# jmhb0/view_neti

Hardware: AMD Instinct MI355X
Metric: TI train steps/sec (SD-1.5 512^2 bs=4 per GPU) (higher is better)
Workload: dtype f16; 1 GPU; learnable_mode 0, sd15 shapes, 512x512 fp16, bs=4/GPU, grad_accum 1, full train step (VAE+16xCLIP+UNet fwd/bwd+AdamW); global_batch=4, parallelism=dp1, rccl_ranks=1, hipgraph=True

## Files before the change

### view_neti_amd/csrc/gemm8.hip

```cpp
#include <type_traits>

#include "common.h"
#include "gemm_args.h"

namespace {

constexpr int BM = 256, NT = 512;
constexpr int HALF_BYTES = 128 * 128;
constexpr int GN_IMG = 5;

#define VN_WAIT_VM(n) asm volatile("s_waitcnt vmcnt(" #n ")" ::: "memory")
#define VN_WAIT_LGKM0() asm volatile("s_waitcnt lgkmcnt(0)" ::: "memory")

template <int BN, int EPI, bool CONV, bool HALO = false>
__global__ __launch_bounds__(NT) void gemm8_kernel(GemmArgs g) {
  static_assert(BN == 256 || BN == 128, "tile width");
  static_assert(!HALO || (BN == 128 && CONV), "the halo-patch loop exists for the 256x128 convolution tile");
  constexpr int PATCH_STRIDE = 41 * 1024;
  constexpr bool H42 = HALO && BN == 128;
  constexpr int NJB = BN / 128;
  constexpr int HB_BYTES = (BN / 2) * 128;
  constexpr int HB_DMA = BN / 128;
  constexpr int NBUF = BN == 256 ? 2 : 3;
  constexpr int BUF_BYTES = 2 * HALF_BYTES + 2 * HB_BYTES;
  constexpr int CS_LD = BN + 8;
  constexpr int CS_BYTES = BM * CS_LD * 2;
  constexpr int LOOP_BYTES = HALO ? 2 * PATCH_STRIDE + 3 * 2 * HB_BYTES : NBUF * BUF_BYTES;
  constexpr int LDS_BYTES = CS_BYTES > LOOP_BYTES ? CS_BYTES : LOOP_BYTES;
  constexpr int GN_NG = BN / 4 + 2;
  const half_t* const e_gate = EPI == 2 ? g.gate_src : nullptr;
  half_t* const e_C2 = EPI == 2 ? g.C2 : nullptr;
  const int e_geglu = EPI == 2 ? g.geglu : 0;
  const int e_act = EPI == 2 ? g.act : 0;
  float* const e_gn_sums = EPI >= 1 ? g.gn_sums : nullptr;
  const half_t* const e_rowadd = EPI >= 1 ? g.rowadd : nullptr;
  const int e_conv = CONV ? g.conv_mode : 0;
  constexpr int GN_BYTES = EPI == 0 ? 0 : GN_IMG * GN_NG * 4 * 8;
  __shared__ __attribute__((aligned(16))) char smem[LDS_BYTES + GN_BYTES];

  const int tid = threadIdx.x;
  const int lane = tid & 63;
  const int wave = __builtin_amdgcn_readfirstlane(tid >> 6);
  const int wr = wave >> 2, wc = wave & 3;

  int nblk = g.tiles_m * g.tiles_n;
  int bid = blockIdx.x;
  {
    int q = nblk >> 3, r = nblk & 7, xcd = bid & 7, idx = bid >> 3;
    bid = (xcd < r ? xcd * (q + 1) : r * (q + 1) + (xcd - r) * q) + idx;
  }
  const int tile_m = bid / g.tiles_n;
  const int tile_n = bid - tile_m * g.tiles_n;
  const int m0 = tile_m * BM;
  const int n0 = tile_n * BN;
  const int bz = blockIdx.y;
  const int kz = blockIdx.z;
  int hb = 0, hty = 0, htx = 0, row0 = m0;
  if constexpr (HALO) {
    const int tpr = g.Wo >> 4, tpi = (g.Ho >> 4) * tpr;
    hb = tile_m / tpi;
    const int rem = tile_m - hb * tpi;
    hty = rem / tpr;
    htx = rem - hty * tpr;
    row0 = (hb * g.Ho + hty * 16) * g.Wo + htx * 16;
  }
  auto rowmem = [&](const int r) { return HALO ? row0 + (r >> 4) * g.Wo + (r & 15) : m0 + r; };

  const half_t* Ab = g.A + (long long)bz * g.strideA;
  const half_t* Bb = g.B + (long long)bz * g.strideB;
  const __amdgpu_buffer_rsrc_t rsA = vn_make_rsrc(Ab, g.a_bytes);
  const __amdgpu_buffer_rsrc_t rsB = vn_make_rsrc(Bb, g.b_bytes);

  const int lrow = tid >> 3;
  const int gchunk = (tid & 7) ^ ((lrow >> 1) & 7);
  const float rcp_hw = CONV ? 1.0f / (float)(g.Ho * g.Wo) : 0.f, rcp_wo = CONV ? 1.0f / (float)g.Wo : 0.f;
  int a_base[4];
  uint32_t a_mask[4];
#pragma unroll
  for (int r = 0; r < (HALO ? 0 : 4); ++r) {
    const int m = m0 + (r >> 1) * 128 + (r & 1) * 64 + lrow;
    const bool ok = m < g.M;
    if constexpr (!CONV) {
      a_base[r] = (int)((long long)m * g.lda * 2) + gchunk * 16;
      a_mask[r] = ok ? 1u : 0u;
    } else {
      const int hw = g.Ho * g.Wo;
      int b = (int)((float)m * rcp_hw);
      int rem = m - b * hw;
      if (rem < 0) { b -= 1; rem += hw; } else if (rem >= hw) { b += 1; rem -= hw; }
      int oy = (int)((float)rem * rcp_wo);
      int ox = rem - oy * g.Wo;
      if (ox < 0) { oy -= 1; ox += g.Wo; } else if (ox >= g.Wo) { oy += 1; ox -= g.Wo; }
      const int py = e_conv == 1 ? oy * g.stride - g.pad_t : oy + g.pad_t;
      const int px = e_conv == 1 ? ox * g.stride - g.pad_l : ox + g.pad_l;
      a_base[r] = ((b * g.Hi + py) * g.Wi + px) * g.ldx2 + gchunk * 16;
      const int sgn = e_conv == 1 ? 1 : -1;
      uint32_t colbits = 0, mask = 0;
#pragma unroll
      for (int d = 0; d < 3; ++d) colbits |= ((unsigned)(px + sgn * d) < (unsigned)g.Wi ? 1u : 0u) << d;
#pragma unroll
      for (int d = 0; d < 3; ++d) mask |= ((unsigned)(py + sgn * d) < (unsigned)g.Hi ? colbits : 0u) << (3 * d);
      a_mask[r] = ok ? mask : 0u;
    }
  }
  uint32_t b_base[4];
#pragma unroll
  for (int r = 0; r < 4; ++r) {
    const int n = n0 + (r >> 1) * (BN / 2) + (r & 1) * 64 + lrow;
    b_base[r] = (n < g.N) ? (uint32_t)((long long)n * g.ldb * 2) + gchunk * 16 : VN_OOB;
  }

  const int nk_total = g.K / 64;
  const int kt_begin = kz * g.kt_per_split;
  const int kt_end = min(nk_total, kt_begin + g.kt_per_split);
  const int T = kt_end - kt_begin;

  int a_kt[2] = {kt_begin, kt_begin}, b_kt[2] = {kt_begin, kt_begin};
  int a_tap[2], a_ci0[2];
  {
    int tap = 0, ci0 = 0;
    if constexpr (CONV) {
      if (g.korder) {
        ci0 = (kt_begin / 9) * 64;
        tap = kt_begin - (kt_begin / 9) * 9;
      } else {
        tap = (kt_begin * 64) / g.Ci;
        ci0 = kt_begin * 64 - tap * g.Ci;
      }
    }
    a_tap[0] = a_tap[1] = tap;
    a_ci0[0] = a_ci0[1] = ci0;
  }
  const int tap_step = (e_conv == 2 ? -1 : 1) * g.ldx2;
  uint32_t nxt[4];
  auto prepA = [&](const int h) {
    const bool live = a_kt[h] < kt_end;
    int soff;
    uint32_t tapbit;
    if constexpr (!CONV) {
      soff = a_kt[h] * 128;
      tapbit = live ? 1u : 0u;
    } else {
      const int tap = a_tap[h];
      const int dy = (tap * 11) >> 5;
      const int dx = tap - 3 * dy;
      soff = (dy * g.Wi + dx) * tap_step + a_ci0[h] * 2;
      tapbit = live ? (1u << tap) : 0u;
      if (g.korder) {
        a_tap[h] += 1;
        if (a_tap[h] == 9) {
          a_tap[h] = 0;
          a_ci0[h] += 64;
        }
      } else {
        a_ci0[h] += 64;
        if (a_ci0[h] == g.Ci) {
          a_ci0[h] = 0;
          a_tap[h] += 1;
        }
      }
    }
#pragma unroll
    for (int j = 0; j < 2; ++j) {
      nxt[j] = (a_mask[2 * h + j] & tapbit) ? (uint32_t)(a_base[2 * h + j] + soff) : VN_OOB;
    }
    a_kt[h] += 1;
  };
  auto prepB = [&](const int h) {
    const bool live = b_kt[h] < kt_end;
    const uint32_t soff = (uint32_t)b_kt[h] * 128u, dead = live ? 0u : VN_OOB;
    if constexpr (BN == 256) {
#pragma unroll
      for (int j = 0; j < 2; ++j) nxt[j] = (b_base[2 * h + j] + soff) | dead;
    } else {
      nxt[2 + h] = (b_base[2 * h] + soff) | dead;
    }
    b_kt[h] += 1;
  };
  auto issueA = [&](const int h, const int buf) {
    char* dst = smem + buf * BUF_BYTES + h * HALF_BYTES + wave * 1024;
#pragma unroll
    for (int j = 0; j < 2; ++j)
      dma16(rsA, dst + j * 8192, nxt[j]);
  };
  auto issueB = [&](const int h, const int buf) {
    char* dst = smem + buf * BUF_BYTES + 2 * HALF_BYTES + h * HB_BYTES + wave * 1024;
    if constexpr (BN == 256) {
#pragma unroll
      for (int j = 0; j < 2; ++j) dma16(rsB, dst + j * 8192, nxt[j]);
    } else {
      dma16(rsB, dst, nxt[2 + h]);
    }
  };

  const int frow = lane & 15;
  const int fq = lane >> 4;
  const int fkey = (frow >> 1) & 7;
  int rdA[2], rdB[2];
#pragma unroll
  for (int s = 0; s < 2; ++s) {
    const int ch = ((s * 4 + fq) ^ fkey) << 4;
    rdA[s] = (wr * 64 + frow) * 128 + ch;
    rdB[s] = 2 * HALF_BYTES + (wc * (16 * NJB) + frow) * 128 + ch;
  }
  half8 af[4][2], bf0[NJB][2], bf1[NJB][2];
  auto readA = [&](const int h) {
#pragma unroll
    for (int i = 0; i < 4; ++i)
#pragma unroll
      for (int s = 0; s < 2; ++s)
        af[i][s] = as_half8(*reinterpret_cast<const u32x4*>(smem + rdA[s] + h * HALF_BYTES + i * 2048));
  };
  auto readB0 = [&](const int flip) {
#pragma unroll
    for (int jb = 0; jb < NJB; ++jb)
#pragma unroll
      for (int s = 0; s < 2; ++s)
        bf0[jb][s] = as_half8(*reinterpret_cast<const u32x4*>(smem + (rdB[s] ^ flip) + jb * 2048));
  };
  auto readB1 = [&]() {
#pragma unroll
    for (int jb = 0; jb < NJB; ++jb)
#pragma unroll
      for (int s = 0; s < 2; ++s)
        bf1[jb][s] = as_half8(*reinterpret_cast<const u32x4*>(smem + rdB[s] + HB_BYTES + jb * 2048));
  };

  const int wr4 = wave >> 1, wc2 = wave & 1;
  auto acc_row = [&](const int h, const int i) { return H42 ? wr4 * 64 + i * 16 + frow : h * 128 + wr * 64 + i * 16 + frow; };
  auto acc_col = [&](const int h, const int j, const int jb) {
    return H42 ? wc2 * 64 + (2 * h + j) * 16 + 4 * fq : j * (BN / 2) + wc * (16 * NJB) + jb * 16 + 4 * fq;
  };
  f32x4 bv[H42 ? 2 : 1][2][NJB];
  {
    const __amdgpu_buffer_rsrc_t rsBias = vn_make_rsrc(g.bias, g.bias ? (uint32_t)g.N * 4u : 0u);
#pragma unroll
    for (int h = 0; h < (H42 ? 2 : 1); ++h)
#pragma unroll
      for (int j = 0; j < 2; ++j)
#pragma unroll
        for (int jb = 0; jb < NJB; ++jb)
          bv[h][j][jb] = __builtin_bit_cast(f32x4, vn_buf_load16(rsBias, (uint32_t)(n0 + acc_col(h, j, jb)) * 4u));
  }
  f32x4 acc[2][2][4][NJB];
#pragma unroll
  for (int h = 0; h < 2; ++h)
#pragma unroll
    for (int j = 0; j < 2; ++j)
#pragma unroll
      for (int i = 0; i < 4; ++i)
#pragma unroll
        for (int jb = 0; jb < NJB; ++jb) acc[h][j][i][jb] = f32x4{0.f, 0.f, 0.f, 0.f};

#define VN_MMA(H, J, BF, PREP)                                                                                 \
  do {                                                                                                         \
    VN_WAIT_LGKM0();                                                                                           \
    __builtin_amdgcn_s_setprio(1);                                                                             \
    PREP;                                                                                                      \
    _Pragma("unroll") for (int s = 0; s < 2; ++s) _Pragma("unroll") for (int i = 0; i < 4; ++i)                \
        _Pragma("unroll") for (int jb = 0; jb < NJB; ++jb) acc[H][J][i][jb] =                                  \
            VN_MFMA_16x16x32(BF[jb][s], af[i][s], acc[H][J][i][jb], 0, 0, 0);                                  \
    __builtin_amdgcn_s_setprio(0);                                                                             \
  } while (0)
#define VN_PHASE_SYNC()                    \
  do {                                     \
    VN_WAIT_VM(10);                        \
    __builtin_amdgcn_s_barrier();          \
    __builtin_amdgcn_sched_barrier(0);     \
  } while (0)
#define VN_PHASE_END()                     \
  do {                                     \
    __builtin_amdgcn_s_barrier();          \
    __builtin_amdgcn_sched_barrier(0);     \
  } while (0)

#define VN_MMA2(H, PREP)                                                                                       \
  do {                                                                                                         \
    VN_WAIT_LGKM0();                                                                                           \
    __builtin_amdgcn_s_setprio(1);                                                                             \
    PREP;                                                                                                      \
    _Pragma("unroll") for (int s = 0; s < 2; ++s) _Pragma("unroll") for (int i = 0; i < 4; ++i) {              \
      acc[H][0][i][0] = VN_MFMA_16x16x32(bf0[0][s], af[i][s], acc[H][0][i][0], 0, 0, 0);                       \
      acc[H][1][i][0] = VN_MFMA_16x16x32(bf1[0][s], af[i][s], acc[H][1][i][0], 0, 0, 0);                       \
    }                                                                                                          \
    __builtin_amdgcn_s_setprio(0);                                                                             \
  } while (0)
#define VN_SYNC(n)                         \
  do {                                     \
    VN_WAIT_VM(n);                         \
    __builtin_amdgcn_s_barrier();          \
    __builtin_amdgcn_sched_barrier(0);     \
  } while (0)
  if constexpr (HALO) {
    constexpr int BRING = 2 * PATCH_STRIDE;
    auto patch_key = [](const int px) { return (int)((0x270745032ull >> (4 * (px >> 1))) & 7); };
    constexpr int PROW = 18 * 128;
    const int c_begin = kt_begin / 9, c_end = kt_end / 9;
    uint32_t pa_off[6];
#pragma unroll
    for (int j = 0; j < 6; ++j) {
      const int q = (j * 8 + wave) * 64 + lane, p = q >> 3, cs = q & 7;
      const int py = (p * 3641) >> 16;
      const int px = p - py * 18;
      const int iy = hty * 16 + py - 1, ix = htx * 16 + px - 1;
      const bool ok = p < 324 && (unsigned)iy < (unsigned)g.Hi && (unsigned)ix < (unsigned)g.Wi;
      pa_off[j] = ok ? (uint32_t)(((hb * g.Hi + iy) * g.Wi + ix) * g.ldx2 + ((cs ^ patch_key(px)) << 4)) : VN_OOB;
    }
    const int np_wave = wave == 0 ? 6 : 5;
    auto issueP = [&](const int j, const int chunk) {
      dma16(rsA, smem + (chunk & 1) * PATCH_STRIDE + (j * 8 + wave) * 1024, pa_off[j] + (uint32_t)chunk * 128u);
    };
    auto tap_dy = [&](const int tap) { const int dy = (tap * 11) >> 5; return e_conv == 2 ? 2 - dy : dy; };
    auto tap_dx = [&](const int tap) { const int dx = tap - 3 * ((tap * 11) >> 5); return e_conv == 2 ? 2 - dx : dx; };
    {
      constexpr int BBUF = 2 * HB_BYTES;
      auto issueBt = [&](const int kt, const int buf) {
        const uint32_t soff = (uint32_t)(kt_begin + kt) * 128u, dead = kt < T ? 0u : VN_OOB;
        char* dst = smem + BRING + buf * BBUF + wave * 1024;
        dma16(rsB, dst, (b_base[0] + soff) | dead);
        dma16(rsB, dst + HB_BYTES, (b_base[2] + soff) | dead);
      };
      int lb[3];
#pragma unroll
      for (int dx = 0; dx < 3; ++dx) lb[dx] = (wr4 * 4) * PROW + (frow + dx) * 128 + ((fq ^ patch_key(frow + dx)) << 4);
      const int rb0 = (wc2 * 64 + frow) * 128 + ((fq ^ fkey) << 4);
      half8 bfh[4][2];
      auto readAh = [&](const int half, const int ab) {
#pragma unroll
        for (int i = 2 * half; i < 2 * half + 2; ++i) {
          af[i][0] = as_half8(*reinterpret_cast<const u32x4*>(smem + ab + i * PROW));
          af[i][1] = as_half8(*reinterpret_cast<const u32x4*>(smem + (ab ^ 64) + i * PROW));
        }
      };
#define VN_MMA4(HALF, PREP)                                                                                    \
  do {                                                                                                         \
    VN_WAIT_LGKM0();                                                                                           \
    __builtin_amdgcn_s_setprio(1);                                                                             \
    PREP;                                                                                                      \
    _Pragma("unroll") for (int s = 0; s < 2; ++s) _Pragma("unroll") for (int i = 2 * HALF; i < 2 * HALF + 2; ++i) \
        _Pragma("unroll") for (int cb = 0; cb < 4; ++cb) {                                                     \
      acc[cb >> 1][cb & 1][i][0] =                                                                             \
          VN_MFMA_16x16x32(bfh[cb][s], af[i][s], acc[cb >> 1][cb & 1][i][0], 0, 0, 0);                         \
    }                                                                                                          \
    __builtin_amdgcn_s_setprio(0);                                                                             \
  } while (0)
      int abt[9];
#pragma unroll
      for (int k = 0; k < 9; ++k) {
        const int tp = e_conv == 2 ? 8 - k : k, dy = tp / 3, dx = tp - 3 * dy;
        abt[k] = (dx == 0 ? lb[0] : (dx == 1 ? lb[1] : lb[2])) + dy * PROW + (c_begin & 1) * PATCH_STRIDE;
      }
      uint32_t bo0 = b_base[0] + (uint32_t)(kt_begin + 2) * 128u, bo1 = b_base[2] + (uint32_t)(kt_begin + 2) * 128u;
      uint32_t pp[6];
#pragma unroll
      for (int j = 0; j < 6; ++j) pp[j] = pa_off[j] + (uint32_t)(c_begin + 1) * 128u;
      const bool w0 = wave == 0;
      char* const bring = smem + BRING + wave * 1024;
      auto readBh = [&](const int slot) {
        const char* b = smem + BRING + slot * BBUF;
#pragma unroll
        for (int cb = 0; cb < 4; ++cb) {
          bfh[cb][0] = as_half8(*reinterpret_cast<const u32x4*>(b + cb * 2048 + rb0));
          bfh[cb][1] = as_half8(*reinterpret_cast<const u32x4*>(b + cb * 2048 + (rb0 ^ 64)));
        }
      };
#pragma unroll
      for (int j = 0; j < 6; ++j)
        if (j < np_wave) issueP(j, c_begin);
      issueBt(0, 0);
      issueBt(1, 1);
      VN_WAIT_VM(2);
      __builtin_amdgcn_s_barrier();
      __builtin_amdgcn_sched_barrier(0);
      if (wr == 1) __builtin_amdgcn_s_barrier();
      __builtin_amdgcn_sched_barrier(0);
      auto ktile = [&](auto tap_c, const bool last_chunk, const int pslot) {
        constexpr int tap = decltype(tap_c)::value;
        constexpr int rslot = tap % 3, sslot = (tap + 2) % 3;
        const int ab = abt[tap];
        readBh(rslot);
        readAh(0, ab);
        if constexpr (tap >= 1 && tap <= 6) {
          if (tap < 6 || w0) {
            dma16(rsA, smem + pslot + ((tap - 1) * 8) * 1024 + wave * 1024, last_chunk ? VN_OOB : pp[tap - 1]);
          }
        }
        {
          const uint32_t dead = (last_chunk && tap >= 7) ? VN_OOB : 0u;
          dma16(rsB, bring + sslot * BBUF, bo0 | dead);
          dma16(rsB, bring + sslot * BBUF + HB_BYTES, bo1 | dead);
          bo0 += 128u;
          bo1 += 128u;
        }
        __builtin_amdgcn_s_barrier();
        __builtin_amdgcn_sched_barrier(0);
        VN_MMA4(0, (void)0);
        VN_PHASE_END();
        readAh(1, ab);
        if constexpr (tap >= 1 && tap <= 5) {
          VN_SYNC(3);
        } else if constexpr (tap == 6) {
          if (w0) {
            VN_SYNC(3);
          } else {
            VN_SYNC(2);
          }
        } else {
          VN_SYNC(2);
        }
        VN_MMA4(1, (void)0);
        VN_PHASE_END();
      };
      for (int c = c_begin; c < c_end; ++c) {
        const bool last_chunk = c + 1 >= c_end;
        const int pslot = ((c + 1) & 1) * PATCH_STRIDE;
        ktile(std::integral_constant<int, 0>{}, last_chunk, pslot);
        ktile(std::integral_constant<int, 1>{}, last_chunk, pslot);
        ktile(std::integral_constant<int, 2>{}, last_chunk, pslot);
        ktile(std::integral_constant<int, 3>{}, last_chunk, pslot);
        ktile(std::integral_constant<int, 4>{}, last_chunk, pslot);
        ktile(std::integral_constant<int, 5>{}, last_chunk, pslot);
        ktile(std::integral_constant<int, 6>{}, last_chunk, pslot);
        ktile(std::integral_constant<int, 7>{}, last_chunk, pslot);
        ktile(std::integral_constant<int, 8>{}, last_chunk, pslot);
        const int flip = (c & 1) ? -PATCH_STRIDE : PATCH_STRIDE;
#pragma unroll
        for (int k = 0; k < 9; ++k) abt[k] += flip;
#pragma unroll
        for (int j = 0; j < 6; ++j) pp[j] += 128u;
      }
#undef VN_MMA4
    }
  } else if constexpr (BN == 256) {
    prepB(0);
    issueB(0, 0);
    prepA(0);
    issueA(0, 0);
    prepB(1);
    issueB(1, 0);
    prepA(1);
    issueA(1, 0);
    prepB(0);
    issueB(0, 1);
    prepA(0);
    issueA(0, 1);
    prepB(1);
    issueB(1, 1);
    prepA(1);
    VN_WAIT_VM(10);
    __builtin_amdgcn_s_barrier();
    __builtin_amdgcn_sched_barrier(0);
    readB0(0);
    VN_WAIT_LGKM0();
    __builtin_amdgcn_sched_barrier(0);
    if (wr == 1) __builtin_amdgcn_s_barrier();
    __builtin_amdgcn_sched_barrier(0);

    int cur = 0;
    for (int t = 0; t < T; ++t) {
      readA(0);
      issueA(1, cur ^ 1);
      VN_PHASE_SYNC();
      VN_MMA(0, 0, bf0, prepB(0));
      VN_PHASE_END();
      readB1();
      issueB(0, cur);
      VN_PHASE_SYNC();
      VN_MMA(0, 1, bf1, prepA(0));
      VN_PHASE_END();
      readA(1);
      issueA(0, cur);
      VN_PHASE_SYNC();
      VN_MMA(1, 0, bf0, prepB(1));
      VN_PHASE_END();
      readB0(BUF_BYTES);
      issueB(1, cur);
      VN_PHASE_SYNC();
      VN_MMA(1, 1, bf1, prepA(1));
      VN_PHASE_END();
      cur ^= 1;
#pragma unroll
      for (int s = 0; s < 2; ++s) {
        rdA[s] ^= BUF_BYTES;
        rdB[s] ^= BUF_BYTES;
      }
    }
  } else {
#pragma unroll
    for (int t0 = 0; t0 < 2; ++t0) {
      prepA(0);
      prepB(0);
      prepB(1);
      issueA(0, t0);
      issueB(0, t0);
      issueB(1, t0);
      prepA(1);
      issueA(1, t0);
    }
    prepA(0);
    prepB(0);
    prepB(1);
    VN_WAIT_VM(8);
    __builtin_amdgcn_s_barrier();
    __builtin_amdgcn_sched_barrier(0);
    if (wr == 1) __builtin_amdgcn_s_barrier();
    __builtin_amdgcn_sched_barrier(0);
    int stg = 2;
    for (int t = 0; t < T; ++t) {
      readB0(0);
      readB1();
      readA(0);
      issueA(0, stg);
      issueB(0, stg);
      issueB(1, stg);
      VN_SYNC(10);
      VN_MMA2(0, prepA(1));
      VN_PHASE_END();
      readA(1);
      issueA(1, stg);
      VN_SYNC(8);
      VN_MMA2(1, (prepA(0), prepB(0), prepB(1)));
      VN_PHASE_END();
      stg = stg == 2 ? 0 : stg + 1;
#pragma unroll
      for (int s = 0; s < 2; ++s) {
        rdA[s] = rdA[s] >= 2 * BUF_BYTES ? rdA[s] - 2 * BUF_BYTES : rdA[s] + BUF_BYTES;
        rdB[s] = rdB[s] >= 2 * BUF_BYTES ? rdB[s] - 2 * BUF_BYTES : rdB[s] + BUF_BYTES;
      }
    }
#undef VN_MMA2
#undef VN_SYNC
  }
  if (wr == 0) __builtin_amdgcn_s_barrier();
  asm volatile("s_waitcnt vmcnt(0) lgkmcnt(0)" ::: "memory");
  __syncthreads();
#undef VN_MMA
#undef VN_PHASE_SYNC
#undef VN_PHASE_END

  if (g.ksplit > 1) {
    float* ws = g.ws + ((long long)(kz * g.batch + bz) * g.M) * g.N;
    const __amdgpu_buffer_rsrc_t rsW = vn_make_rsrc(ws, 0x7fffffffu);
#pragma unroll
    for (int h = 0; h < 2; ++h)
#pragma unroll
      for (int j = 0; j < 2; ++j)
#pragma unroll
        for (int i = 0; i < 4; ++i)
#pragma unroll
          for (int jb = 0; jb < NJB; ++jb) {
            const int m = rowmem(acc_row(h, i));
            const int n = n0 + acc_col(h, j, jb);
            if (m < g.M && n < g.N) {
              float* p = ws + (long long)m * g.N + n;
              if (n + 4 <= g.N && (g.N & 3) == 0) {
                vn_st16_wt(rsW, (uint32_t)(((long long)m * g.N + n) * 4), acc[h][j][i][jb]);
              } else {
                for (int e = 0; e < 4 && n + e < g.N; ++e) p[e] = acc[h][j][i][jb][e];
              }
            }
          }
    return;
  }

  if (e_gn_sums && !(HALO && g.gn_hw == g.Ho * g.Wo)) {
    vn_u64* gacc = reinterpret_cast<vn_u64*>(smem + LDS_BYTES);
    for (int i = tid; i < GN_IMG * GN_NG * 4; i += NT) gacc[i] = 0;
  }
  {
    const int nsw = ((frow >> 3) & 1) << 2;
#pragma unroll
    for (int h = 0; h < 2; ++h)
#pragma unroll
      for (int i = 0; i < 4; ++i)
#pragma unroll
        for (int j = 0; j < 2; ++j)
#pragma unroll
          for (int jb = 0; jb < NJB; ++jb) {
            const int ml = acc_row(h, i);
            const int nl = acc_col(h, j, jb) ^ nsw;
            half4 o;
#pragma unroll
            for (int e = 0; e < 4; ++e)
              o[e] = (half_t)apply_act(acc[h][j][i][jb][e] * g.alpha + bv[H42 ? h : 0][j][jb][e], e_act);
            *reinterpret_cast<half4*>(smem + ((size_t)ml * CS_LD + nl) * 2) = o;
          }
  }
  __syncthreads();

  half_t* Cb = reinterpret_cast<half_t*>(g.C) + (long long)bz * g.strideC;
  const __amdgpu_buffer_rsrc_t rsC = vn_make_rsrc(Cb, 0x7fffffffu);
  const __amdgpu_buffer_rsrc_t rsC2 = vn_make_rsrc(e_C2, e_C2 ? 0x7fffffffu : 0u);
  const half_t* Rb = reinterpret_cast<const half_t*>(g.resid);
  if (Rb) Rb += (long long)bz * g.strideC;
  constexpr int CPR = BN / 8;
  constexpr int U = EPI == 2 ? 2 : (EPI == 1 ? 4 : (BN == 256 ? 8 : 4));
  static_assert(NT % CPR == 0 && CPR <= 32 && (BM * CPR) % NT == 0, "a thread keeps one 8-column chunk over all its rows");
  vn_u64* gacc = reinterpret_cast<vn_u64*>(smem + LDS_BYTES);
  const bool gn = e_gn_sums != nullptr;
  const float rcp_gnhw = gn ? 1.0f / (float)g.gn_hw : 0.f, rcp_rpg = e_rowadd ? 1.0f / (float)g.rows_per_group : 0.f;
  const int gn_img0 = gn ? row0 / g.gn_hw : 0, gn_g0t = gn ? n0 / g.gn_cpg : 0;
  const int c = (tid % CPR) * 8;
  const int n = n0 + c;
  const int gn_glo = gn ? n / g.gn_cpg : 0;
  const int gn_split = gn ? (gn_glo + 1) * g.gn_cpg - n : 8;
  int gn_img = -1;
  float s_lo = 0.f, q_lo = 0.f, s_hi = 0.f, q_hi = 0.f;
  auto gn_flush = [&]() {
    const int iref = __builtin_amdgcn_readfirstlane(gn_img);
    const bool uni = __all(gn_img == iref) && iref >= 0;
    if (uni) {
#pragma unroll
      for (int off = 32; off >= CPR; off >>= 1) {
        s_lo += __shfl_xor(s_lo, off);
        q_lo += __shfl_xor(q_lo, off);
        s_hi += __shfl_xor(s_hi, off);
        q_hi += __shfl_xor(q_hi, off);
      }
    }
    if (gn_img >= 0 && (!uni || lane < CPR)) {
      vn_u64* a = gacc + ((gn_img - gn_img0) * GN_NG + (gn_glo - gn_g0t)) * 4;
      vn_fx_add2(a, s_lo, q_lo);
      if (gn_split < 8) vn_fx_add2(a + 4, s_hi, q_hi);
    }
    s_lo = q_lo = s_hi = q_hi = 0.f;
  };
  const bool full_chunk = n + 8 <= g.N;
  const bool swap_halves = ((tid / CPR) >> 3) & 1;
  const __amdgpu_buffer_rsrc_t rsR = vn_make_rsrc(Rb, Rb ? 0x7fffffffu : 0u);
  const __amdgpu_buffer_rsrc_t rsRA = vn_make_rsrc(e_rowadd, e_rowadd ? 0x7fffffffu : 0u);
  const __amdgpu_buffer_rsrc_t rsG = vn_make_rsrc(e_gate, e_gate ? 0x7fffffffu : 0u);
  const int r_first = tid / CPR;
  constexpr int RPP = NT / CPR;
  const bool gn_one = HALO && gn && g.gn_hw == g.Ho * g.Wo;
  const bool ra_one = HALO && EPI >= 1 && e_rowadd && g.rows_per_group == g.Ho * g.Wo;
  half8 av_tile = half8{0, 0, 0, 0, 0, 0, 0, 0};
  if (ra_one) av_tile = as_half8(vn_buf_load16(rsRA, full_chunk ? (uint32_t)(((long long)hb * g.ld_rowadd + n) * 2) : VN_OOB));
  if (gn_one) gn_img = hb;
  for (int it0 = 0; it0 < BM / RPP; it0 += U) {
    half8 cv[U], rv[U], av[U], gv[U], gv2[U];
#pragma unroll
    for (int u = 0; u < U; ++u) {
      const int r = r_first + RPP * (it0 + u);
      const int m = rowmem(r);
      const bool ok = m < g.M && full_chunk;
      u32x4 t = *reinterpret_cast<const u32x4*>(smem + ((size_t)r * CS_LD + c) * 2);
      if (swap_halves) t = u32x4{t[2], t[3], t[0], t[1]};
      cv[u] = as_half8(t);
      if (Rb) rv[u] = as_half8(vn_buf_load16(rsR, ok ? (uint32_t)(((long long)m * g.ldr + n) * 2) : VN_OOB));
      if (EPI >= 1) {
        if (ra_one) {
          av[u] = av_tile;
        } else if (e_rowadd) {
          int grp = (int)((float)m * rcp_rpg);
          const int rem = m - grp * g.rows_per_group;
          grp += rem >= g.rows_per_group ? 1 : (rem < 0 ? -1 : 0);
          av[u] = as_half8(vn_buf_load16(rsRA, ok ? (uint32_t)(((long long)grp * g.ld_rowadd + n) * 2) : VN_OOB));
        }
      }
      if (EPI == 2 && e_gate) {
        const long long go = (long long)m * g.ld_gate + (e_geglu == 2 ? 2 * n : n);
        gv[u] = as_half8(vn_buf_load16_once(rsG, ok ? (uint32_t)(go * 2) : VN_OOB));
        gv2[u] = as_half8(vn_buf_load16_once(rsG, (ok && e_geglu == 2) ? (uint32_t)(go * 2 + 16) : VN_OOB));
      }
    }
#pragma unroll
    for (int u = 0; u < U; ++u) {
      const int r = r_first + RPP * (it0 + u);
      const int m = rowmem(r);
      const bool valid = m < g.M && n < g.N;
      if (gn && !gn_one) {
        int img = gn_img;
        if (valid) {
          img = (int)((float)m * rcp_gnhw);
          const int rem = m - img * g.gn_hw;
          img += rem >= g.gn_hw ? 1 : (rem < 0 ? -1 : 0);
        }
        if (__any(img != gn_img)) {
          gn_flush();
          gn_img = img;
        }
      }
      if (!valid) continue;
      half8 v = cv[u];
      if (full_chunk) {
        if (EPI >= 1 && e_rowadd) {
          v = vn_add8(v, av[u]);
        }
        if (Rb) {
          v = vn_add8(v, rv[u]);
        }
        if (e_geglu == 2) {
#pragma unroll
          for (int c2 = 0; c2 < 2; ++c2) {
            const half8 pre = c2 == 0 ? gv[u] : gv2[u];
            half8 o;
#pragma unroll
            for (int e = 0; e < 4; ++e) {
              const float d = (float)v[4 * c2 + e], hh = (float)pre[e], gg = (float)pre[4 + e];
              float cdf, xpdf;
              vn_gelu_parts(gg, cdf, xpdf);
              o[e] = (half_t)(d * gg * cdf);
              o[4 + e] = (half_t)(d * hh * (cdf + xpdf));
            }
            vn_st16_wt(rsC, (uint32_t)(((long long)m * g.ldc + 2 * n + 8 * c2) * 2), o);
          }
          continue;
        }
        if (e_gate) {
#pragma unroll
          for (int e = 0; e < 8; ++e) v[e] = (half_t)((float)v[e] * act_grad((float)gv[u][e], g.gate_act));
        }
        if (e_geglu == 1 || (e_C2 && e_geglu == 0)) vn_st16_wt_saved(rsC, (uint32_t)(((long long)m * g.ldc + n) * 2), v);
        else vn_st16_wt(rsC, (uint32_t)(((long long)m * g.ldc + n) * 2), v);
        if (e_geglu == 1) {
          half4 o2;
#pragma unroll
          for (int e = 0; e < 4; ++e) o2[e] = (half_t)((float)v[e] * vn_gelu_erf((float)v[4 + e]));
          *reinterpret_cast<half4*>(e_C2 + (long long)m * g.ldc2 + (n >> 1)) = o2;
        }
        if (gn) {
          {
            const half2v one2 = {(half_t)1.f, (half_t)1.f};
#pragma unroll
            for (int e = 0; e < 8; e += 2) {
              const half2v p2 = {v[e], v[e + 1]};
              if (e < gn_split) {
                s_lo = VN_FDOT2(p2, one2, s_lo);
                q_lo = VN_FDOT2(p2, p2, q_lo);
              } else {
                s_hi = VN_FDOT2(p2, one2, s_hi);
                q_hi = VN_FDOT2(p2, p2, q_hi);
              }
            }
          }
        }
        if (e_C2 && e_geglu == 0) {
          half8 o2;
#pragma unroll
          for (int e = 0; e < 8; ++e) o2[e] = (half_t)apply_act((float)v[e], g.act2);
          vn_st16_wt(rsC2, (uint32_t)(((long long)m * g.ldc2 + n) * 2), o2);
        }
      } else {
        const half_t* radd = e_rowadd ? e_rowadd + (long long)(m / g.rows_per_group) * g.ld_rowadd + n : nullptr;
        for (int e = 0; e < 8 && n + e < g.N; ++e) {
          float x = (float)v[e];
          if (radd) x = (float)(half_t)(x + (float)radd[e]);
          if (Rb) x = (float)(half_t)(x + (float)Rb[(long long)m * g.ldr + n + e]);
          if (e_gate) x = (float)(half_t)(x * act_grad((float)e_gate[(long long)m * g.ld_gate + n + e], g.gate_act));
          Cb[(long long)m * g.ldc + n + e] = (half_t)x;
          if (e_C2) e_C2[(long long)m * g.ldc2 + n + e] = (half_t)apply_act((float)(half_t)x, g.act2);
          if (gn) {
            const float xs = (float)(half_t)x;
            if (e < gn_split) {
              s_lo += xs;
              q_lo += xs * xs;
            } else {
              s_hi += xs;
              q_hi += xs * xs;
            }
          }
        }
      }
    }
  }
  if (gn_one) {
    float v4[4] = {s_lo, q_lo, s_hi, q_hi};
#pragma unroll
    for (int k = 0; k < 4; ++k) {
      v4[k] += __shfl_xor(v4[k], 32);
      v4[k] += __shfl_xor(v4[k], 16);
    }
    static_assert(CPR == 16 || !HALO, "the halo tile is 128 columns wide");
    float* tab = reinterpret_cast<float*>(smem + LDS_BYTES);
    if (lane < 16) *reinterpret_cast<f32x4*>(tab + (wave * 16 + lane) * 4) = f32x4{v4[0], v4[1], v4[2], v4[3]};
    __syncthreads();
    if (tid < 32) {
      const int col = tid >> 1, half = tid & 1;
      float sv = 0.f, qv = 0.f;
#pragma unroll
      for (int w8 = 0; w8 < 8; ++w8) {
        sv += tab[(w8 * 16 + col) * 4 + 2 * half];
        qv += tab[(w8 * 16 + col) * 4 + 2 * half + 1];
      }
      const int nc = n0 + col * 8;
      const int glo = nc / g.gn_cpg;
      const int split = (glo + 1) * g.gn_cpg - nc;
      if (nc < g.N && (half == 0 || split < 8)) {
        const int slot = tile_m % g.gn_slots;
        vn_u64* dst = reinterpret_cast<vn_u64*>(e_gn_sums) + (((long long)hb * g.gn_slots + slot) * g.gn_G + glo + half) * 4;
        vn_fx_add2(dst, sv, qv);
      }
    }
  } else if (gn) {
    gn_flush();
    __syncthreads();
    const int slot = tile_m % g.gn_slots;
    for (int i = tid; i < GN_IMG * GN_NG; i += NT) {
      const vn_u64* src = gacc + 4 * i;
      if ((src[0] | src[1] | src[2] | src[3]) == 0) continue;
      const int img = gn_img0 + i / GN_NG, grp = gn_g0t + i % GN_NG;
      vn_u64* dst = reinterpret_cast<vn_u64*>(e_gn_sums) + (((long long)img * g.gn_slots + slot) * g.gn_G + grp) * 4;
#pragma unroll
      for (int w = 0; w < 4; ++w) atomicAdd(dst + w, src[w]);
    }
  }
}

inline int epilogue_level8(const GemmArgs& g) {
  if (g.gate_src || g.C2 || g.geglu || g.act) return 2;
  return (g.gn_sums || g.rowadd) ? 1 : 0;
}

}

int vneti_launch_gemm8(void* gemm_args, int bn, int halo, hipStream_t st) {
  GemmArgs& g = *reinterpret_cast<GemmArgs*>(gemm_args);
  if (g.out_f32 || (g.conv_mode && (g.ups || (g.conv_mode == 2 && g.stride == 2))) ||
      (g.M >= (1 << 24) && (g.conv_mode || g.rowadd || g.gn_sums)))
    return VNETI_EUNSUP;
  if (halo && (bn != 128 || g.conv_mode < 1 || g.conv_mode > 2 || g.stride != 1 || g.pad_t != 1 || g.pad_l != 1 || g.Hi != g.Ho ||
               g.Wi != g.Wo || (g.Ho & 15) || (g.Wo & 15) || (g.Ci & 63) || g.K != 9 * g.Ci || !g.korder ||
               g.batch != 1 || g.M != (g.M / (g.Ho * g.Wo)) * g.Ho * g.Wo))
    return VNETI_EUNSUP;
  if (halo && g.ksplit > 1) {
    const int nchunk = g.Ci / 64, cps = cdiv(nchunk, g.ksplit);
    g.kt_per_split = 9 * cps;
    g.ksplit = cdiv(nchunk, cps);
  }
  g.tiles_m = cdiv(g.M, BM);
  g.tiles_n = cdiv(g.N, bn);
  const dim3 grid(g.tiles_m * g.tiles_n, g.batch, g.ksplit), block(NT);
  const int epi = epilogue_level8(g);
#define VN_GO(E, C)                                                                        \
  do {                                                                                     \
    if (bn == 256) hipLaunchKernelGGL((gemm8_kernel<256, E, C>), grid, block, 0, st, g);   \
    else hipLaunchKernelGGL((gemm8_kernel<128, E, C>), grid, block, 0, st, g);             \
  } while (0)
#define VN_GO_HALO(E) hipLaunchKernelGGL((gemm8_kernel<128, E, true, true>), grid, block, 0, st, g)
  if (halo) {
    if (epi == 2) VN_GO_HALO(2); else if (epi == 1) VN_GO_HALO(1); else VN_GO_HALO(0);
  } else if (g.conv_mode) {
    if (epi == 2) VN_GO(2, true); else if (epi == 1) VN_GO(1, true); else VN_GO(0, true);
  } else {
    if (epi == 2) VN_GO(2, false); else if (epi == 1) VN_GO(1, false); else VN_GO(0, false);
  }
#undef VN_GO
#undef VN_GO_HALO
  return vneti_check_launch("gemm8_kernel");
}
```

Baseline: 40.05 steps/s.

## Reorder conv taps column-major to reuse A-fragment registers across dy shifts

The halo-patch convolution loop now visits the nine taps column by column (dx outer, dy inner) instead of row-major. It keeps a sliding window of six A fragment rows in registers, so each tap loads only the one new row instead of re-reading four rows from LDS. B-tile prefetch offsets and the generic prep paths are remapped through small permutation tables to match the new tap order. The aim is to cut LDS read traffic and waits in the inner MFMA loop, at the cost of more registers for the window and more complex index logic.

After: 40.22 steps/s (median of 6 runs). Within noise of the previous version (+0.4%).

```diff
diff --git a/view_neti_amd/csrc/gemm8.hip b/view_neti_amd/csrc/gemm8.hip
--- a/view_neti_amd/csrc/gemm8.hip
+++ b/view_neti_amd/csrc/gemm8.hip
@@ -117,6 +117,10 @@
 
   int a_kt[2] = {kt_begin, kt_begin}, b_kt[2] = {kt_begin, kt_begin};
   int a_tap[2], a_ci0[2];
+  int b_sh[2] = {0, 0};
+  const bool cm = CONV && g.korder;
+  const unsigned long long ptab = cm ? 0x852741630ull : 0x876543210ull;
+  const unsigned long long dtab = cm ? 0x420642864ull : 0x444444444ull;
   {
     int tap = 0, ci0 = 0;
     if constexpr (CONV) {
@@ -130,6 +134,7 @@
     }
     a_tap[0] = a_tap[1] = tap;
     a_ci0[0] = a_ci0[1] = ci0;
+    if (cm) b_sh[0] = b_sh[1] = 4 * tap;
   }
   const int tap_step = (e_conv == 2 ? -1 : 1) * g.ldx2;
   uint32_t nxt[4];
@@ -141,7 +146,7 @@
       soff = a_kt[h] * 128;
       tapbit = live ? 1u : 0u;
     } else {
-      const int tap = a_tap[h];
+      const int tap = (int)(ptab >> (4 * a_tap[h])) & 15;
       const int dy = (tap * 11) >> 5;
       const int dx = tap - 3 * dy;
       soff = (dy * g.Wi + dx) * tap_step + a_ci0[h] * 2;
@@ -168,7 +173,12 @@
   };
   auto prepB = [&](const int h) {
     const bool live = b_kt[h] < kt_end;
-    const uint32_t soff = (uint32_t)b_kt[h] * 128u, dead = live ? 0u : VN_OOB;
+    int kt = b_kt[h];
+    if constexpr (CONV) {
+      kt += ((int)(dtab >> b_sh[h]) & 15) - 4;
+      b_sh[h] = b_sh[h] == 32 ? 0 : b_sh[h] + 4;
+    }
+    const uint32_t soff = (uint32_t)kt * 128u, dead = live ? 0u : VN_OOB;
     if constexpr (BN == 256) {
 #pragma unroll
       for (int j = 0; j < 2; ++j) nxt[j] = (b_base[2 * h + j] + soff) | dead;
@@ -325,32 +335,30 @@
       for (int dx = 0; dx < 3; ++dx) lb[dx] = (wr4 * 4) * PROW + (frow + dx) * 128 + ((fq ^ patch_key(frow + dx)) << 4);
       const int rb0 = (wc2 * 64 + frow) * 128 + ((fq ^ fkey) << 4);
       half8 bfh[4][2];
-      auto readAh = [&](const int half, const int ab) {
-#pragma unroll
-        for (int i = 2 * half; i < 2 * half + 2; ++i) {
-          af[i][0] = as_half8(*reinterpret_cast<const u32x4*>(smem + ab + i * PROW));
-          af[i][1] = as_half8(*reinterpret_cast<const u32x4*>(smem + (ab ^ 64) + i * PROW));
-        }
+      half8 aw[6][2];
+      auto readW = [&](const int w, const int ab0, const int ab1) {
+        aw[w][0] = as_half8(*reinterpret_cast<const u32x4*>(smem + ab0 + w * PROW));
+        aw[w][1] = as_half8(*reinterpret_cast<const u32x4*>(smem + ab1 + w * PROW));
       };
-#define VN_MMA4(HALF, PREP)                                                                                    \
+#define VN_MMA4(HALF, DY)                                                                                      \
   do {                                                                                                         \
     VN_WAIT_LGKM0();                                                                                           \
     __builtin_amdgcn_s_setprio(1);                                                                             \
-    PREP;                                                                                                      \
-    _Pragma("unroll") for (int s = 0; s < 2; ++s) _Pragma("unroll") for (int i = 2 * HALF; i < 2 * HALF + 2; ++i) \
+    _Pragma("unroll") for (int s = 0; s < 2; ++s) _Pragma("unroll") for (int i = 2 * (HALF); i < 2 * (HALF) + 2; ++i) \
         _Pragma("unroll") for (int cb = 0; cb < 4; ++cb) {                                                     \
       acc[cb >> 1][cb & 1][i][0] =                                                                             \
-          VN_MFMA_16x16x32(bfh[cb][s], af[i][s], acc[cb >> 1][cb & 1][i][0], 0, 0, 0);                         \
+          VN_MFMA_16x16x32(bfh[cb][s], aw[i + (DY)][s], acc[cb >> 1][cb & 1][i][0], 0, 0, 0);                  \
     }                                                                                                          \
     __builtin_amdgcn_s_setprio(0);                                                                             \
   } while (0)
-      int abt[9];
-#pragma unroll
-      for (int k = 0; k < 9; ++k) {
-        const int tp = e_conv == 2 ? 8 - k : k, dy = tp / 3, dx = tp - 3 * dy;
-        abt[k] = (dx == 0 ? lb[0] : (dx == 1 ? lb[1] : lb[2])) + dy * PROW + (c_begin & 1) * PATCH_STRIDE;
-      }
-      uint32_t bo0 = b_base[0] + (uint32_t)(kt_begin + 2) * 128u, bo1 = b_base[2] + (uint32_t)(kt_begin + 2) * 128u;
+      int abx[3][2];
+#pragma unroll
+      for (int d = 0; d < 3; ++d) {
+        const int dx = e_conv == 2 ? 2 - d : d;
+        abx[d][0] = (dx == 0 ? lb[0] : (dx == 1 ? lb[1] : lb[2])) + (c_begin & 1) * PATCH_STRIDE;
+        abx[d][1] = abx[d][0] ^ 64;
+      }
+      uint32_t bo0 = b_base[0] + (uint32_t)(kt_begin + 6) * 128u, bo1 = b_base[2] + (uint32_t)(kt_begin + 6) * 128u;
       uint32_t pp[6];
 #pragma unroll
       for (int j = 0; j < 6; ++j) pp[j] = pa_off[j] + (uint32_t)(c_begin + 1) * 128u;
@@ -368,38 +376,52 @@
       for (int j = 0; j < 6; ++j)
         if (j < np_wave) issueP(j, c_begin);
       issueBt(0, 0);
-      issueBt(1, 1);
+      issueBt(3, 1);
       VN_WAIT_VM(2);
       __builtin_amdgcn_s_barrier();
       __builtin_amdgcn_sched_barrier(0);
       if (wr == 1) __builtin_amdgcn_s_barrier();
       __builtin_amdgcn_sched_barrier(0);
-      auto ktile = [&](auto tap_c, const bool last_chunk, const int pslot) {
-        constexpr int tap = decltype(tap_c)::value;
-        constexpr int rslot = tap % 3, sslot = (tap + 2) % 3;
-        const int ab = abt[tap];
+      auto ktile = [&](auto pos_c, auto dg_c, const bool last_chunk, const int pslot) {
+        constexpr int pos = decltype(pos_c)::value;
+        constexpr bool DG = decltype(dg_c)::value;
+        constexpr int rslot = pos % 3, sslot = (pos + 2) % 3;
+        constexpr int col = pos / 3, dyw = DG ? 2 - pos % 3 : pos % 3;
+        constexpr int h0 = DG ? 1 : 0;
+        constexpr int inew = DG ? 0 : 3;
+        constexpr int stage_now = 9 * ((pos + 2) / 9) + 3 * ((pos + 2) % 9 % 3) + (pos + 2) % 9 / 3;
+        constexpr int stage_nxt = 9 * ((pos + 3) / 9) + 3 * ((pos + 3) % 9 % 3) + (pos + 3) % 9 / 3;
+        const int ab0 = abx[col][0], ab1 = abx[col][1];
         readBh(rslot);
-        readAh(0, ab);
-        if constexpr (tap >= 1 && tap <= 6) {
-          if (tap < 6 || w0) {
-            dma16(rsA, smem + pslot + ((tap - 1) * 8) * 1024 + wave * 1024, last_chunk ? VN_OOB : pp[tap - 1]);
+        if constexpr (pos % 3 == 0) {
+          readW(2 * h0 + dyw, ab0, ab1);
+          readW(2 * h0 + dyw + 1, ab0, ab1);
+        }
+        if constexpr (pos >= 1 && pos <= 6) {
+          if (pos < 6 || w0) {
+            dma16(rsA, smem + pslot + ((pos - 1) * 8) * 1024 + wave * 1024, last_chunk ? VN_OOB : pp[pos - 1]);
           }
         }
         {
-          const uint32_t dead = (last_chunk && tap >= 7) ? VN_OOB : 0u;
+          const uint32_t dead = (last_chunk && pos >= 7) ? VN_OOB : 0u;
           dma16(rsB, bring + sslot * BBUF, bo0 | dead);
           dma16(rsB, bring + sslot * BBUF + HB_BYTES, bo1 | dead);
-          bo0 += 128u;
-          bo1 += 128u;
+          bo0 += (uint32_t)((stage_nxt - stage_now) * 128);
+          bo1 += (uint32_t)((stage_nxt - stage_now) * 128);
         }
         __builtin_amdgcn_s_barrier();
         __builtin_amdgcn_sched_barrier(0);
-        VN_MMA4(0, (void)0);
+        VN_MMA4(h0, dyw);
         VN_PHASE_END();
-        readAh(1, ab);
-        if constexpr (tap >= 1 && tap <= 5) {
+        if constexpr (pos % 3 == 0) {
+          readW(2 * (1 - h0) + dyw, ab0, ab1);
+          readW(2 * (1 - h0) + dyw + 1, ab0, ab1);
+        } else {
+          readW(inew + dyw, ab0, ab1);
+        }
+        if constexpr (pos >= 1 && pos <= 5) {
           VN_SYNC(3);
-        } else if constexpr (tap == 6) {
+        } else if constexpr (pos == 6) {
           if (w0) {
             VN_SYNC(3);
           } else {
@@ -408,27 +430,34 @@
         } else {
           VN_SYNC(2);
         }
-        VN_MMA4(1, (void)0);
+        VN_MMA4(1 - h0, dyw);
         VN_PHASE_END();
       };
-      for (int c = c_begin; c < c_end; ++c) {
-        const bool last_chunk = c + 1 >= c_end;
-        const int pslot = ((c + 1) & 1) * PATCH_STRIDE;
-        ktile(std::integral_constant<int, 0>{}, last_chunk, pslot);
-        ktile(std::integral_constant<int, 1>{}, last_chunk, pslot);
-        ktile(std::integral_constant<int, 2>{}, last_chunk, pslot);
-        ktile(std::integral_constant<int, 3>{}, last_chunk, pslot);
-        ktile(std::integral_constant<int, 4>{}, last_chunk, pslot);
-        ktile(std::integral_constant<int, 5>{}, last_chunk, pslot);
-        ktile(std::integral_constant<int, 6>{}, last_chunk, pslot);
-        ktile(std::integral_constant<int, 7>{}, last_chunk, pslot);
-        ktile(std::integral_constant<int, 8>{}, last_chunk, pslot);
-        const int flip = (c & 1) ? -PATCH_STRIDE : PATCH_STRIDE;
-#pragma unroll
-        for (int k = 0; k < 9; ++k) abt[k] += flip;
-#pragma unroll
-        for (int j = 0; j < 6; ++j) pp[j] += 128u;
-      }
+      auto chunks = [&](auto dg_c) {
+        for (int c = c_begin; c < c_end; ++c) {
+          const bool last_chunk = c + 1 >= c_end;
+          const int pslot = ((c + 1) & 1) * PATCH_STRIDE;
+          ktile(std::integral_constant<int, 0>{}, dg_c, last_chunk, pslot);
+          ktile(std::integral_constant<int, 1>{}, dg_c, last_chunk, pslot);
+          ktile(std::integral_constant<int, 2>{}, dg_c, last_chunk, pslot);
+          ktile(std::integral_constant<int, 3>{}, dg_c, last_chunk, pslot);
+          ktile(std::integral_constant<int, 4>{}, dg_c, last_chunk, pslot);
+          ktile(std::integral_constant<int, 5>{}, dg_c, last_chunk, pslot);
+          ktile(std::integral_constant<int, 6>{}, dg_c, last_chunk, pslot);
+          ktile(std::integral_constant<int, 7>{}, dg_c, last_chunk, pslot);
+          ktile(std::integral_constant<int, 8>{}, dg_c, last_chunk, pslot);
+          const int flip = (c & 1) ? -PATCH_STRIDE : PATCH_STRIDE;
+#pragma unroll
+          for (int d = 0; d < 3; ++d) {
+            abx[d][0] += flip;
+            abx[d][1] += flip;
+          }
+#pragma unroll
+          for (int j = 0; j < 6; ++j) pp[j] += 128u;
+        }
+      };
+      if (e_conv == 2) chunks(std::true_type{});
+      else chunks(std::false_type{});
 #undef VN_MMA4
     }
   } else if constexpr (BN == 256) {
```
